# young-how/DQN-based-UAV-3D_path_planer

Measured on AMD Instinct MI355X. Metric: env-steps/sec + learner updates/sec, PathPlan_City DQN, higher is better.
Workload: dtype f64

## Files before the change

dqn_based_uav_3d_path_planer_amd/csrc/learner.hip:

```cpp
#include <hip/hip_runtime.h>
#include <hip/hip_fp16.h>
#include <stdint.h>
#include <stdlib.h>

#include "../../include/uavenv.h"
#include "uavenv_device.hpp"
#include "qnet_device.hpp"
#include "dqn_internal.hpp"
#include "dqn_slots_internal.hpp"

using namespace uav;
using namespace uavq;

namespace {

struct GradArgs {
    UavReplayRing ring;
    int head, filled, batch;
    uint64_t seed, counter;
    ReplayPerm perm;
    const int32_t *explicit_idx;
    const float *local, *target;
    int n_actions, dueling, kind;
    float gamma;
// ... 685 lines not shown
            csc = mfma16(ones ? 1.0f : xs[q][i], dh[q][i], csc);
            cw2 = mfma16(hh[q][i], bo[q][i], cw2);
        }
#pragma unroll
    for (int k = 0; k < 4; ++k) { A.acc[0][k] += csc[k]; A.acc[1][k] += cw2[k]; }
}

template <bool FIRST, bool GLDS>
__device__ __forceinline__ void grad_tile_packed8(const GradArgs &g, const GradLdsP &L, float *qn_lds, int tile, bool more,
                                                  GradAcc8 &A)
{
    constexpr int NMAX = 4;
    const int tid = (int)threadIdx.x, lane = tid & 63, wv = __builtin_amdgcn_readfirstlane(tid >> 6), grp = wv >> 2, strip = wv & 3;
    const int r = lane & 15, gq = lane >> 4, t256 = tid & 255;
    const int n2 = g.n_actions + (g.dueling ? 1 : 0);
    const uint32_t *obs = reinterpret_cast<const uint32_t *>(g.ring.obs);
    const float *net = grp == 0 ? g.local : g.target;
    floatx4 vW[kStageIters];
    SplitScRegs vS;
    float pw[4] = {0, 0, 0, 0}, pb2 = 0.0f;
    if (FIRST) {
        if (GLDS) img_glds(grp == 0 ? L.W1l : L.W1t, g.img + (grp == 0 ? 0 : kSplitF), strip);
        else if (g.img) img_issue(vW, g.img + (grp == 0 ? 0 : kSplitF));
        else w_issue_half(vW, net, t256);
        const NetDev nv = net_view(net, n2);
        if (!GLDS && !g.img) w_issue_sc(vS, net, nv.b1);
#pragma unroll
        for (int k = 0; k < 4; ++k) pw[k] = nv.W2[t256 + 256 * k < n2 * kHid ? t256 + 256 * k : 0];
        pb2 = nv.b2[t256 < n2 ? t256 : 0];
    }
    L_STAMP2(0);
    const int smp = tile * kTile + strip * 16 + r;
    int f, agent;
    if (g.explicit_idx) {
        f = g.explicit_idx[2 * smp];
        agent = g.explicit_idx[2 * smp + 1];
    } else {
        replay_slot_to_frame(g.perm, replay_perm_apply(g.perm, (uint32_t)smp), g.head, g.ring.frames, f, agent);
    }
    int fn = f + 1;
    if (fn >= g.ring.frames) fn = 0;
    const uint32_t row_s = (uint32_t)f * (uint32_t)g.ring.n_agents + (uint32_t)agent;
    const uint32_t row_n = (uint32_t)fn * (uint32_t)g.ring.n_agents + (uint32_t)agent;
    L_STAMP2(1);
    PRow R;
    prow_load(R, obs + (size_t)(grp == 0 ? row_s : row_n) * kPackedDwords);
    int p_act = 0;
    float p_rew = 0.0f, p_w = 1.0f;
    uint32_t raw_done = 0u, raw_valid = 1u;
    if (grp == 0) {
        load_transition(g.ring, row_s, p_act, p_rew, raw_done, raw_valid);
        p_w = g.is_w ? g.is_w[smp] : 1.0f;
    }
    L_STAMP(6);
    if (FIRST) {
        if (!GLDS) {
            if (g.img) img_commit(grp == 0 ? L.W1l : L.W1t, vW); else w_commit_split(w1split_at(grp == 0 ? L.W1l : L.W1t), vW, vS);
        }
        L_STAMP(7);
        float *W2 = grp == 0 ? L.W2l : L.W2t, *b2 = grp == 0 ? L.b2l : L.b2t;
#pragma unroll
        for (int k = 0; k < 4; ++k)
            if (t256 + 256 * k < n2 * kHid) W2[t256 + 256 * k] = pw[k];
        if (t256 < n2) b2[t256] = pb2;
        __syncthreads();
    }
    L_STAMP(1);
    floatx4 hl[4];
    W2Frag<NMAX> Fl;
    float ql[NMAX];
    if (grp == 0) {
        fwd_strip_split<false>(w1split_at(L.W1l), R, hl);
        w2_load<NMAX>(Fl, L.W2l, L.b2l, n2);
        q_strip<NMAX>(hl, Fl, n2, g.n_actions, g.dueling, ql);
        if (gq == 0) prow_store_lds(L.Ps + (strip * 16 + r) * kPackedDwords, R);
    } else {
        int best = 0;
        floatx4 ht[4];
        if (g.kind == 1) {
            fwd_strip_split<false>(w1split_at(L.W1l), R, ht);
            W2Frag<NMAX> F;
            w2_load<NMAX>(F, L.W2l, L.b2l, n2);
            float qn_l[NMAX];
            q_strip<NMAX>(ht, F, n2, g.n_actions, g.dueling, qn_l);
            float bq = qn_l[0];
#pragma unroll
            for (int a = 1; a < NMAX; ++a)
                if (a < g.n_actions && qn_l[a] > bq) { bq = qn_l[a]; best = a; }
        }
        fwd_strip_split<false>(w1split_at(L.W1t), R, ht);
        W2Frag<NMAX> Ft;
        w2_load<NMAX>(Ft, L.W2t, L.b2t, n2);
        float qt[NMAX];
        q_strip<NMAX>(ht, Ft, n2, g.n_actions, g.dueling, qt);
        if (gq == 0) qn_lds[strip * 16 + r] = pick_qn<NMAX>(g, qt, best);
    }
    L_STAMP(2);
    __syncthreads();
    L_STAMP(3);
    FlagOps FO;
    if (grp == 1) flag_ops_build(L, r, gq, FO);
    if (grp == 0) {
        GradAcc<NMAX> T;
#pragma unroll
        for (int a = 0; a < NMAX + 2; ++a) T.csum[a] = A.csum[a];
        float amax = 0.0f;
// ... 510 lines not shown
                if (grp == 0) A.acc[3] = mfma16h(*reinterpret_cast<const half8 *>(xa + 16 * 6 * kLdT + 32 * kk), bdh, A.acc[3]);
                else A.acc[3] = mfma16h(*reinterpret_cast<const half8 *>(ha + 32 * kk), *reinterpret_cast<const half8 *>(ob + 32 * kk), A.acc[3]);
            }
        }
        if (i + 1 < n_my) __syncthreads();
    }
    L_STAMP(5);
    grad_write_partials8(g, ga.stride, red, A);
}

constexpr size_t kGradH8Lds = (size_t)(4 * kTile * kLdH + 2 * kTile * kLdT + 2 * 112 * kLdT + 16 * kLdT) * 2 +
                              (size_t)(2 * kMaxOut * kHid + 2 * kMaxOut + 4 * (kMaxOut + 2) + 2 * kTile + 8 * kStageW) * 4;

template <typename ObsT, int NMAX>
__global__ void __launch_bounds__(256) k_dqn_grad(Grad2Args ga)
{
    const GradArgs &g = ga.g;
    extern __shared__ __align__(16) float lds[];
    GradLds L;
    L.W1l = lds;
    L.W1t = L.W1l + kTileF;
    L.Xs = L.W1t + kTileF;
    L.Xn = L.Xs + kTileF;
    L.dHs = L.Xn + kTileF;
    L.douts = L.dHs + kTile * kLh;
    L.W2l = L.douts + kTile * kMaxOut;
    L.W2t = L.W2l + kMaxOut * kHid;
    L.b2l = L.W2t + kMaxOut * kHid;
    L.b2t = L.b2l + kMaxOut;
    L.red = L.b2t + kMaxOut;
    const int tid = (int)threadIdx.x, lane = tid & 63, wv = tid >> 6, r = lane & 15, gq = lane >> 4;
    const int n2 = g.n_actions + (g.dueling ? 1 : 0);
    GradAcc<NMAX> A;
    A.acc2 = floatx4{0.0f, 0.0f, 0.0f, 0.0f};
#pragma unroll
    for (int u = 0; u < 7; ++u) A.acc1[u] = floatx4{0.0f, 0.0f, 0.0f, 0.0f};
#pragma unroll
    for (int a = 0; a < NMAX + 2; ++a) A.csum[a] = 0.0f;

    L_STAMP(0);
    const int step = (int)gridDim.x;
    int tile = (int)blockIdx.x;
    grad_tile<ObsT, NMAX, true>(g, L, tile, tile + step < ga.n_tiles, A);
    for (tile += step; tile < ga.n_tiles; tile += step)
        grad_tile<ObsT, NMAX, false>(g, L, tile, tile + step < ga.n_tiles, A);
    L_STAMP(5);
    grad_write_partials<NMAX>(g, ga.stride, L.red, A);
}

constexpr int kMaxGradGrid = 256;
constexpr size_t kGrad2Lds = (size_t)(4 * kTileF + kTile * kLh + kTile * kMaxOut + 2 * kMaxOut * kHid + 2 * kMaxOut +
                                      4 * (kMaxOut + 2)) * 4;

__device__ __forceinline__ float reduce_columns(const float *__restrict__ partials, int nblk, int P, int stride, float &c_out)
{
    __shared__ float red[32][33];
    __shared__ float red2[8][33];
    const int tid = (int)threadIdx.x;
    const int cg = tid & 7, rg = tid >> 3;
    const int p4 = (int)blockIdx.x * 32 + cg * 4;
    const bool col_ok = p4 < stride;
    floatx4 acc = floatx4{0.0f, 0.0f, 0.0f, 0.0f};
    float c = 0.0f;
    for (int b0 = 0; b0 < nblk; b0 += 256) {
        floatx4 t[8];
#pragma unroll
        for (int k = 0; k < 8; ++k) {
            const int b = b0 + rg + 32 * k;
            const int bb = b < nblk ? b : nblk - 1;
            t[k] = *reinterpret_cast<const floatx4 *>(partials + (size_t)bb * stride + (col_ok ? p4 : 0));
        }
        const int bc = b0 + tid;
        const float cv = partials[(size_t)(bc < nblk ? bc : nblk - 1) * stride + P + 1];
        c += bc < nblk ? cv : 0.0f;
#pragma unroll
        for (int k = 0; k < 8; ++k) {
            const bool ok = b0 + rg + 32 * k < nblk;
#pragma unroll
            for (int e = 0; e < 4; ++e) acc[e] += ok ? t[k][e] : 0.0f;
        }
    }
    c_out = c;
#pragma unroll
    for (int e = 0; e < 4; ++e) red[rg][cg * 4 + e] = acc[e];
    __syncthreads();
    {
        const int px = tid & 31, part = tid >> 5;
        red2[part][px] = (red[4 * part][px] + red[4 * part + 1][px]) + (red[4 * part + 2][px] + red[4 * part + 3][px]);
    }
    __syncthreads();
    float t = 0.0f;
    if (tid < 32) {
#pragma unroll
        for (int k = 0; k < 8; ++k) t += red2[k][tid];
    }
    return t;
}

__global__ void __launch_bounds__(256) k_dqn_reduce(const float *__restrict__ partials, int nblk, int P, int stride,
                                                    float *__restrict__ raw)
{
    float c;
    const float t = reduce_columns(partials, nblk, P, stride, c);
    const int p = (int)blockIdx.x * 32 + (int)threadIdx.x;
    if (threadIdx.x < 32 && p < P + 2) raw[p] = t;
}

__global__ void k_dqn_adam(float *__restrict__ local, float *__restrict__ target, float *__restrict__ m,
                           float *__restrict__ v, const float *__restrict__ raw, int P, float lr, float beta1,
                           float beta2, float eps, float bc1, float bc2_sqrt, int hard_update, float *__restrict__ loss,
                           float *__restrict__ img)
{
    const int p = (int)(blockIdx.x * blockDim.x + threadIdx.x);
    const float cnt = raw[P + 1];
    const float inv = 1.0f / (cnt > 1.0f ? cnt : 1.0f);
    if (p == 0 && loss) *loss = raw[P] * inv;
    if (p >= P) return;
    const float gp = raw[p] * inv;
    const float mp = m[p] + (gp - m[p]) * (1.0f - beta1);
    const float vp = v[p] * beta2 + (1.0f - beta2) * gp * gp;
    m[p] = mp;
    v[p] = vp;
    const float denom = sqrtf(vp) / bc2_sqrt + eps;
    const float np = local[p] - (lr / bc1) * (mp / denom);
    local[p] = np;
    if (hard_update) target[p] = np;
    if (img) {
        img_store_param(img, p, np);
        if (hard_update) img_store_param(img + kSplitF, p, np);
    }
}

__global__ void __launch_bounds__(256) k_dqn_reduce_adam(const float *__restrict__ partials, int nblk, int P, int stride,
                                                         float *__restrict__ local, float *__restrict__ target,
                                                         float *__restrict__ m, float *__restrict__ v, float lr,
                                                         float beta1, float beta2, float eps, float bc1, float bc2_sqrt,
                                                         int hard_update, float *__restrict__ loss, float *__restrict__ raw,
                                                         const uint32_t *__restrict__ go_word, uint32_t go_value, float *__restrict__ img)
{
    UAV_HOT_PRIO();
    if (go_word && __hip_atomic_load(go_word, __ATOMIC_RELAXED, __HIP_MEMORY_SCOPE_AGENT) != go_value) return;
    __shared__ float cnt_part[4];
    const int tid = (int)threadIdx.x;
    const int p = (int)blockIdx.x * 32 + tid;
    float m0 = 0.0f, v0 = 0.0f, w0 = 0.0f;
    if (tid < 32 && p < P) { m0 = m[p]; v0 = v[p]; w0 = local[p]; }
    float c;
    const float t = reduce_columns(partials, nblk, P, stride, c);
    for (int off = 32; off > 0; off >>= 1) c += __shfl_down(c, off, 64);
    if ((tid & 63) == 0) cnt_part[tid >> 6] = c;
    __syncthreads();
    const float cnt = (cnt_part[0] + cnt_part[1]) + (cnt_part[2] + cnt_part[3]);
    const float inv = 1.0f / (cnt > 1.0f ? cnt : 1.0f);
    if (tid < 32 && p < P + 2) {
        if (raw) raw[p] = t;
        if (p < P) {
            const float gp = t * inv;
            const float mp = m0 + (gp - m0) * (1.0f - beta1);
            const float vp = v0 * beta2 + (1.0f - beta2) * gp * gp;
            m[p] = mp;
            v[p] = vp;
            const float np = w0 - (lr / bc1) * (mp / (sqrtf(vp) / bc2_sqrt + eps));
            local[p] = np;
            if (hard_update) target[p] = np;
            if (img) {
                img_store_param(img, p, np);
                if (hard_update) img_store_param(img + kSplitF, p, np);
            }
        } else if (p == P && loss) {
            *loss = t * inv;
        }
    }
}

struct AdamSlotsArgs {
    int nblk, P, stride;
    float lr, beta1, beta2, eps;
    const uint32_t *go_word;
    uint32_t go_value;
    struct {
        const float *partials;
        float *local, *target, *m, *v, *loss, *raw, *img;
        float bc1, bc2_sqrt;
        int hard_update;
    } slot[kActMaxSlots];
};

__global__ void __launch_bounds__(256) k_dqn_reduce_adam_slots(AdamSlotsArgs a)
{
    const auto &sl = a.slot[blockIdx.y];
    const float *__restrict__ partials = sl.partials;
    float *__restrict__ local = sl.local, *__restrict__ target = sl.target, *__restrict__ m = sl.m, *__restrict__ v = sl.v;
    float *__restrict__ loss = sl.loss, *__restrict__ raw = sl.raw, *__restrict__ img = sl.img;
    const uint32_t *__restrict__ go_word = a.go_word;
    const uint32_t go_value = a.go_value;
    const int nblk = a.nblk, P = a.P, stride = a.stride, hard_update = sl.hard_update;
    const float lr = a.lr, beta1 = a.beta1, beta2 = a.beta2, eps = a.eps, bc1 = sl.bc1, bc2_sqrt = sl.bc2_sqrt;
    UAV_HOT_PRIO();
    if (go_word && __hip_atomic_load(go_word, __ATOMIC_RELAXED, __HIP_MEMORY_SCOPE_AGENT) != go_value) return;
    __shared__ float cnt_part[4];
    const int tid = (int)threadIdx.x;
    const int p = (int)blockIdx.x * 32 + tid;
    float m0 = 0.0f, v0 = 0.0f, w0 = 0.0f;
    if (tid < 32 && p < P) { m0 = m[p]; v0 = v[p]; w0 = local[p]; }
    float c;
    const float t = reduce_columns(partials, nblk, P, stride, c);
    for (int off = 32; off > 0; off >>= 1) c += __shfl_down(c, off, 64);
    if ((tid & 63) == 0) cnt_part[tid >> 6] = c;
    __syncthreads();
    const float cnt = (cnt_part[0] + cnt_part[1]) + (cnt_part[2] + cnt_part[3]);
    const float inv = 1.0f / (cnt > 1.0f ? cnt : 1.0f);
    if (tid < 32 && p < P + 2) {
        if (raw) raw[p] = t;
        if (p < P) {
            const float gp = t * inv;
            const float mp = m0 + (gp - m0) * (1.0f - beta1);
            const float vp = v0 * beta2 + (1.0f - beta2) * gp * gp;
            m[p] = mp;
            v[p] = vp;
            const float np = w0 - (lr / bc1) * (mp / (sqrtf(vp) / bc2_sqrt + eps));
            local[p] = np;
            if (hard_update) target[p] = np;
            if (img) {
                img_store_param(img, p, np);
                if (hard_update) img_store_param(img + kSplitF, p, np);
            }
        } else if (p == P && loss) {
            *loss = t * inv;
        }
    }
}

struct ActArgs {
    const void *obs;
    int n, n_actions, dueling;
    const float *local;
    float eps;
    uint64_t seed, counter;
    int32_t *index_out;
    float *steer_out;
    float *q_out;
    const float *img;
};

template <typename ObsT, int NMAX>
__global__ void __launch_bounds__(256) k_dqn_act(ActArgs g)
{
    extern __shared__ __align__(16) float lds[];
    float *W1 = lds;
    float *Xs = W1 + kTileF;
    float *W2 = Xs + kTileF;
    float *b2 = W2 + kMaxOut * kHid;
    const int tid = (int)threadIdx.x, lane = tid & 63, wv = tid >> 6, r = lane & 15;
    const int n2 = g.n_actions + (g.dueling ? 1 : 0);
    const NetDev nl = net_view(g.local, n2);
    const int first = (int)blockIdx.x * kTile + wv * 16;
    float *strip = Xs + wv * kStripF;
    floatx4 vX[kXIters], vW[kStageIters];
    {
// ... 736 lines not shown
```

dqn_based_uav_3d_path_planer_amd/csrc/qnet_device.hpp:

```cpp
#pragma once
#include <hip/hip_runtime.h>
#include <stdint.h>

#include "uavenv_device.hpp"

namespace uavq {

using namespace uav;

constexpr int kW = 100;
constexpr int kHid = 64;
constexpr int kTile = 64;
constexpr int kMaxOut = 16;

struct NetDev {
    const float *W1, *b1, *W2, *b2;
};

__device__ __forceinline__ NetDev net_view(const float *flat, int n2)
{
    NetDev n;
    n.W1 = flat;
    n.b1 = flat + kHid * kW;
    n.W2 = n.b1 + kHid;
// ... 288 lines not shown
#pragma unroll
    for (int it = 0; it < kStageIters; ++it)
#pragma unroll
        for (int e = 0; e < 4; ++e) {
            h[it][e] = (_Float16)v[it][e];
            m[it][e] = (_Float16)((v[it][e] - (float)h[it][e]) * 2048.0f);
        }
#pragma unroll
    for (int it = 0; it < kStageIters; ++it) {
        const int c = it * 256 + tid;
        const int row = c / 25, q = c - row * 25;
        if (c < kStageChunks && q >= 2 && q < 24) {
            *reinterpret_cast<half4 *>(S.hi + row * kLdHs + 4 * q - kFlagC0) = h[it];
            *reinterpret_cast<half4 *>(S.mid + row * kLdHs + 4 * q - kFlagC0) = m[it];
        }
    }
    float *d = S.sc + (tid >> 2) * kScK + 5 * (tid & 3);
#pragma unroll
    for (int i = 0; i < 5; ++i) d[i] = R.v[i];
}
__device__ __forceinline__ void stage_actor_split(const W1Split &S, const float *flat)
{
    floatx4 v[kStageIters];
    SplitScRegs sc;
    w_issue(v, flat);
    w_issue_sc(sc, flat, flat + kHid * kW);
    w_commit_split(S, v, sc);
}
constexpr int kImgPieces = kSplitBytes / 16;
static_assert((kImgPieces + 255) / 256 == kStageIters, "the image is staged through the registers of w_issue");
__device__ __forceinline__ void img_issue(floatx4 (&v)[kStageIters], const float *img)
{
    const int tid = (int)threadIdx.x & 255;
#pragma unroll
    for (int it = 0; it < kStageIters; ++it) {
        int c = it * 256 + tid;
        c = c < kImgPieces ? c : kImgPieces - 1;
        v[it] = *reinterpret_cast<const floatx4 *>(img + 4 * c);
    }
}
__device__ __forceinline__ void img_commit(float *lds_image, const floatx4 (&v)[kStageIters])
{
    const int tid = (int)threadIdx.x & 255;
#pragma unroll
    for (int it = 0; it < kStageIters; ++it) {
        const int c = it * 256 + tid;
        if (c < kImgPieces) *reinterpret_cast<floatx4 *>(lds_image + 4 * c) = v[it];
    }
}
__device__ __forceinline__ void glds16(const void *src, void *lds_base)
{
    __builtin_amdgcn_global_load_lds((__attribute__((address_space(1))) void *)src,
                                     (__attribute__((address_space(3))) void *)lds_base, 16, 0, 0);
}
constexpr int kImgDma = kImgPieces / 64;
static_assert(kImgPieces % 64 == 0 && (kImgDma + 3) / 4 == 7 && kImgDma > 4 * 6, "the image is 27 whole wavefront-instructions");
__device__ __forceinline__ void img_glds(float *lds_image, const float *img, int w)
{
    const int lane = (int)threadIdx.x & 63;
#pragma unroll
    for (int it = 0; it < 6; ++it) {
        const int c = (4 * it + w) * 64;
        glds16(img + 4 * (c + lane), lds_image + 4 * c);
    }
    const int c = (24 + w) * 64;
    if (c < kImgPieces) glds16(img + 4 * (c + lane), lds_image + 4 * c);
}
__device__ __forceinline__ void img_store_param(float *img, int p, float w)
{
    const W1Split S = w1split_at(img);
    if (p < kHid * kW) {
        const int row = p / kW;
        split_store(S, row, p - row * kW, w);
    } else if (p < kHid * kW + kHid) {
        S.sc[(p - kHid * kW) * kScK + 15] = w;
    }
}

__device__ __forceinline__ half8 bits_to_half8(uint32_t byte)
{
    uintx4 d;
#pragma unroll
    for (int k = 0; k < 4; ++k)
        d[k] = ((byte >> (2 * k)) & 1u ? 0x3c00u : 0u) | ((byte >> (2 * k + 1)) & 1u ? 0x3c000000u : 0u);
    return *reinterpret_cast<const half8 *>(&d);
}
__device__ __forceinline__ uint32_t flag_byte(const PRow &R, int kk, int g)
{
    const uint32_t lo = kk == 0 ? R.m0 : (kk == 1 ? R.m1 : R.m2), hi = kk == 0 ? R.m1 : (kk == 1 ? R.m2 : 0u);
    return g == 3 ? (hi & 0xffu) : ((lo >> (8 * (g + 1))) & 0xffu);
}
__device__ __forceinline__ int flag_aoff(int kk, int g)
{
    return (kk == 2 && g == 3) ? 0 : 32 * kk + 8 * g;
}
__device__ __forceinline__ float sel4(float a0, float a1, float a2, float a3, uint32_t m1, uint32_t m2)
{
    const uint32_t lo = (__float_as_uint(a1) & m1) | (__float_as_uint(a0) & ~m1);
    const uint32_t hi = (__float_as_uint(a3) & m1) | (__float_as_uint(a2) & ~m1);
    return __uint_as_float((hi & m2) | (lo & ~m2));
}

template <bool EXT>
__device__ __forceinline__ void fwd_strip_split_ahead(const W1Split &S, const PRow &R, floatx4 (&acc)[4], float e0 = 0.0f, float e1 = 0.0f)
{
    const int lane = (int)threadIdx.x & 63, r = lane & 15, g = lane >> 4;
// ... 265 lines not shown
```

dqn_based_uav_3d_path_planer_amd/csrc/uavenv.hip:

```cpp
#include <hip/hip_runtime.h>

#include <algorithm>
#include <cmath>
#include <cstdarg>
#include <cstdio>
#include <cstdlib>
#include <cstring>
#include <map>
#include <mutex>
#include <new>
#include <utility>
#include <vector>

#include "../../include/uavenv.h"
#include "uavenv_device.hpp"
#include "qnet_device.hpp"
#include "dqn_internal.hpp"

using namespace uav;

extern "C" int uavenv_rrt_plan_at(UavEnv *env, int32_t first, int32_t m, const double *start_goal_dev, const double *uniforms_dev,
                                  int32_t stream_len, uint64_t seed, int32_t max_iter, double step_size, double obstacle_step,
                                  double *out_start_goal_dev, double *out_sub_dev, int32_t *out_nsub_dev,
                                  int32_t *out_iters_dev, void *node_scratch, int32_t scratch_wgs, void *stream);
// ... 979 lines not shown
    const DevState &S = a.st;
    const int N = a.N;
    const int lane = (int)threadIdx.x & 63, wv = __builtin_amdgcn_readfirstlane((int)threadIdx.x >> 6);
    const int first = (int)blockIdx.x * 64;
    const int i = first + lane;
    const bool active = i < N;
    const int ii = active ? i : N - 1;
    CoopLds *C = reinterpret_cast<CoopLds *>(smem + a.obsq_off);
    const bool want_obs = a.obs && !(a.flags & UAVENV_STEP_NO_OBS);
    const bool auto_reset = (a.flags & UAVENV_STEP_AUTO_RESET) != 0;
    UAV_CSTAMP(0);

    const uavq::W1Split pW1 = uavq::w1split_at(reinterpret_cast<float *>(smem + a.pol_off));
    float *pW2 = reinterpret_cast<float *>(smem + a.pol_off) + uavq::kSplitF;
    float *pb2 = pW2 + uavq::kMaxOut * uavq::kHid;
    int32_t *pact = reinterpret_cast<int32_t *>(pb2 + uavq::kMaxOut);
    uavq::floatx4 vW[uavq::kStageIters];
    uavq::PRow prow;
    uavq::SplitScRegs pol_sc;
    float pol_w2[4] = {0, 0, 0, 0}, pol_b2v = 0.0f;
    uint4 pol_rn = make_uint4(0u, 0u, 0u, 0u);
    const int pol_i = first + wv * 16 + (lane & 15);
    const int pol_n2 = a.n_actions + (a.pol_dueling ? 1 : 0);
    if (POLICY) {
        const int tid = (int)threadIdx.x;
        const uavq::NetDev nl = uavq::net_view(a.pol_local, pol_n2);
        if (GLDS) {
            uavq::img_glds(reinterpret_cast<float *>(smem + a.pol_off), a.pol_img, wv);
            if (wv >= 2) stage_copy_glds(smem, a, wv - 2, 2);
        } else if (a.pol_img) uavq::img_issue(vW, a.pol_img);
        else { uavq::w_issue(vW, a.pol_local); uavq::w_issue_sc(pol_sc, a.pol_local, nl.b1); }
#pragma unroll
        for (int k = 0; k < 4; ++k) pol_w2[k] = nl.W2[tid + 256 * k < pol_n2 * uavq::kHid ? tid + 256 * k : pol_n2 * uavq::kHid - 1];
        pol_b2v = nl.b2[tid < pol_n2 ? tid : 0];
        uavq::prow_load(prow, a.pol_obs + (size_t)(pol_i < N ? pol_i : N - 1) * kPackedDwords);
        pol_rn = philox4x32_10(make_uint4((uint32_t)pol_i, (uint32_t)a.pol_counter, (uint32_t)(a.pol_counter >> 32), 0xac7u),
                               make_uint2((uint32_t)a.pol_seed, (uint32_t)(a.pol_seed >> 32)));
    }
    Agent g;
    RawAction ra = {0u, 0u};
    double head_old = 0.0;
    uint32_t meta_a1 = 0u;
    if (wv == 0) {
        load_agent(S, ii, g);
        if (!POLICY) ra = load_action_raw(a.actions, a.action_kind, ii);
        if (a.meta_a1) meta_a1 = __float_as_uint(a.meta_a1[ii]);
    } else if (wv == 2) {
        head_old = S.F(F_HEAD)[ii];
        if (!POLICY) ra = load_action_raw(a.actions, a.action_kind, ii);
    }
    ResetCand cand;
    double cand_heading = 0.0;
    bool cand_want = false;
    if (wv == 1 && auto_reset) {
        const int c_flags = S.I(I_FLAGS)[ii], c_sub = S.I(I_SUBIDX)[ii], c_n = S.I(I_NTOTAL)[ii], c_step = S.I(I_STEP)[ii];
        const double dx = S.F(F_GX)[ii] - S.F(F_PX)[ii], dy = S.F(F_GY)[ii] - S.F(F_PY)[ii],
                     dz = S.F(F_GZ)[ii] - S.F(F_PZ)[ii];
        cand_heading = reset_candidate_draw(a, ii, cand);
        const double reach = 7.0 + a.max_v + 1.0;
        cand_want = (c_flags & kFlagDone) || c_sub >= c_n - 1 || c_step + 1 >= a.max_step ||
                    dx * dx + dy * dy + dz * dz < reach * reach;
        if (cand_want) reset_candidate_fetch(a, cand);
    }
    uint2 lut[7];
    {
        const int lo = wv == 0 ? 0 : 7 + (wv - 1) * 6;
#pragma unroll
        for (int j = 0; j < 6; ++j) lut[j] = a.emit_lut[(lo + j) * 64 + lane];
        lut[6] = a.emit_lut[6 * 64 + lane];
    }
    uint32_t *trow = C->tile + lane * kCTileLd;
    if (wv == 3) { trow[0] = 0u; trow[1] = 0u; trow[2] = 0u; }
    double r = 0.0, a0 = 0.0;
    int ret_done = 0, info = UAVENV_INFO_NORMAL, valid = 1, agent_done = 0;
    double energy = 0.0;
    bool did_reset = false, skip = false, head_set = false;
    PreStep pre;
    pre.moved = false;
    if (POLICY) {
        const int tid = (int)threadIdx.x;
        if (!GLDS) {
            if (a.pol_img) uavq::img_commit(reinterpret_cast<float *>(smem + a.pol_off), vW); else uavq::w_commit_split(pW1, vW, pol_sc);
        }
#pragma unroll
        for (int k = 0; k < 4; ++k) {
            const int at = tid + 256 * k < pol_n2 * uavq::kHid ? tid + 256 * k : pol_n2 * uavq::kHid - 1;
            pW2[at] = pol_w2[k];
        }
        if (tid < pol_n2) pb2[tid] = pol_b2v;
    }
    if (wv >= 2) {
        if (!(POLICY && GLDS)) stage_copy(smem, a, (int)threadIdx.x - 128, 128);
    } else if (wv == 0) {
        unpack_flags(g);
        const bool masked = a.active && a.active[ii] == 0;
        skip = masked || ((a.flags & UAVENV_STEP_SKIP_DONE) && g.done);
        if (!POLICY) {
            a0 = decode_action(ra, a.action_kind, a.n_actions);
            if (!skip) step_pre(a, a0, g, pre);
        }
        else if (!skip) {
            step_pre_dists(g, pre);
        }
    }
    __syncthreads();
    UAV_PSTAMP(1);
    const WorldLds<MaskT> w = world_view<MaskT>(smem, a);
    if (POLICY) {
        uavq::floatx4 h[4];
        uavq::W2Frag<4> F;
        if (PAHEAD) uavq::fwd_strip_split_ahead<false>(pW1, prow, h);
        else uavq::fwd_strip_split<false>(pW1, prow, h);
        UAV_PSTAMP(2);
        float q[4];
        uavq::w2_load<4>(F, pW2, pb2, pol_n2);
        uavq::q_strip<4>(h, F, pol_n2, a.n_actions, a.pol_dueling, q);
        if (lane < 16) {
            const float sample = (float)(pol_rn.x >> 8) * (1.0f / 16777216.0f);
            int act;
            if (sample > a.pol_eps) {
                act = 0;
                float bq = q[0];
#pragma unroll
                for (int k = 1; k < 4; ++k)
                    if (k < a.n_actions && q[k] > bq) { bq = q[k]; act = k; }
            } else {
                act = (int)(((uint64_t)pol_rn.y * (uint64_t)a.n_actions) >> 32);
            }
            pact[wv * 16 + lane] = act;
            if (pol_i < N) a.pol_act[pol_i] = act;
        }
        UAV_PSTAMP(3);
        __syncthreads();
        UAV_PSTAMP(4);
        if (wv == 0 || wv == 2) ra.lo = (uint32_t)pact[lane];
        if (wv == 0) {
            a0 = decode_action(ra, UAVENV_ACT_INDEX_I32, a.n_actions);
            if (!skip && pre.moved) {
                double sn, cs;
                sincos(g.head + a0 * a.steer, &sn, &cs);
                step_pre_move(a, g, pre, sn, cs);
            }
        }
// ... 300 lines not shown
    c.scn = row;
    reset_candidate_fetch(a, c);
    double vx, vy;
    if (v.v0) {
        vx = v.v0[(size_t)L.e * 2];
        vy = v.v0[(size_t)L.e * 2 + 1];
    } else {
        const uint4 r = philox4x32_10(make_uint4((uint32_t)L.e, 0u, 0u, 0xe7a1u), make_uint2((uint32_t)v.seed, (uint32_t)(v.seed >> 32)));
        double sn, cs;
        sincos(kTwoPi * u53(r.x, r.y), &sn, &cs);
        vx = a.max_v * cs;
        vy = a.max_v * sn;
    }
    L.v0x = vx;
    L.v0y = vy;
    c.f[14] = calc_v(vx, vy, a.max_v);
    c.f[12] = vx;
    c.f[13] = vy;
    c.f[15] = angle_of<true>(vx, vy);
    apply_reset<APF>(a, APF ? li : L.e, g, c);
    L.steps = 0;
    L.collisions = 0;
    L.cap = c.n_total * a.max_step + 1;
    L.ret = 0.0;
    L.energy = 0.0;
    if (v.traj_steps > 0) {
        double *p = v.traj_pos + (size_t)L.e * (v.traj_steps + 1) * 3;
        p[0] = g.o.px; p[1] = g.o.py; p[2] = g.o.pz;
    }
}

template <typename MaskT>
__global__ void __launch_bounds__(256, 1) k_eval_episodes(StepArgs a, EvalArgs v)
{
    extern __shared__ __align__(16) unsigned char smem[];
    const int lane = (int)threadIdx.x & 63, wv = __builtin_amdgcn_readfirstlane((int)threadIdx.x >> 6);
    const int tid = (int)threadIdx.x;
    float *img = reinterpret_cast<float *>(smem + v.img_off);
    float *W2 = reinterpret_cast<float *>(smem + v.w2_off);
    float *b2 = W2 + uavq::kMaxOut * uavq::kHid;
    uavq::img_glds(img, v.img, wv);
    if (wv >= 2) stage_copy_glds(smem, a, wv - 2, 2);
    {
        const uavq::NetDev nl = uavq::net_view(v.local, v.n2);
#pragma unroll
        for (int k = 0; k < 4; ++k)
            if (tid + 256 * k < v.n2 * uavq::kHid) W2[tid + 256 * k] = nl.W2[tid + 256 * k];
        if (tid < v.n2) b2[tid] = nl.b2[tid];
    }
    Agent g = {};
    EvalLane L = {};
    L.e = (int)blockIdx.x * 256 + tid;
    bool install = true;
    __syncthreads();
    const WorldLds<MaskT> w = world_view<MaskT>(smem, a);
    const uavq::W1Split W1 = uavq::w1split_at(img);
    unsigned char *slot = smem + v.slot_off + wv * v.slot_bytes;
    ObsWaveLds *Q = reinterpret_cast<ObsWaveLds *>(slot);
    uint32_t *rows = reinterpret_cast<uint32_t *>(slot);
    const int r16 = lane & 15, grp = lane >> 4;
    const int A = a.n_actions;
    for (;;) {
        if (install) eval_install(a, v, g, L);
        install = false;
        if (__ballot(L.e < v.n) == 0ull) break;
        const bool have = L.e < v.n;
        const ObsBits bits = obs_bits_queued(w, Q, g.o.px, g.o.py, g.o.pz, have);
        const ObsScalars sc = obs_scalars(g.o, g.head);
        uavq::PRow R;
        ctile_mask_words(bits, R.m0, R.m1, R.m2);
#pragma unroll
        for (int k = 0; k < 11; ++k) R.sc[k] = sc.f[k];
#pragma unroll
        for (int k = 0; k < 4; ++k) R.sg[k] = sc.f[11 + k];
        if (!have) {
            R.m0 = R.m1 = R.m2 = 0u;
#pragma unroll
            for (int k = 0; k < 11; ++k) R.sc[k] = 0.0f;
#pragma unroll
            for (int k = 0; k < 4; ++k) R.sg[k] = 0.0f;
        }
        wave_lds_sync();
        uavq::prow_store_lds(rows + lane * kPackedDwords, R);
        wave_lds_sync();
        float q[4] = {0.0f, 0.0f, 0.0f, 0.0f};
#pragma unroll 1
        for (int st = 0; st < 4; ++st) {
            uavq::PRow Rs;
            uavq::prow_load(Rs, rows + (16 * st + r16) * kPackedDwords);
            uavq::floatx4 h[4];
            uavq::fwd_strip_split<false>(W1, Rs, h);
            uavq::W2Frag<4> F;
            uavq::w2_load<4>(F, W2, b2, v.n2);
            float qs[4];
            uavq::q_strip<4>(h, F, v.n2, A, v.dueling, qs);
#pragma unroll
            for (int k = 0; k < 4; ++k) q[k] = grp == st ? qs[k] : q[k];
        }
        wave_lds_sync();
        if (have) {
            int act = 0;
            float bq = q[0];
#pragma unroll
            for (int k = 1; k < 4; ++k)
                if (k < A && q[k] > bq) { bq = q[k]; act = k; }
            if (v.eps > 0.0f) {
// ... 43 lines not shown
    float bound;
    int32_t mode, n_actors;
    int32_t n, first, max_steps, traj_steps, lanes;
    int32_t img_off, w2_off, slot_off, slot_bytes;
};

__device__ __forceinline__ float2 eval_sac_noise(uint64_t seed, int e, int step)
{
    const uint4 r = philox4x32_10(make_uint4((uint32_t)e, (uint32_t)step, 0u, 0x5ac0u), make_uint2((uint32_t)seed, (uint32_t)(seed >> 32)));
    const float u1 = ((float)(r.x >> 8) + 1.0f) * (1.0f / 16777216.0f);
    const float u2 = (float)(r.y >> 8) * (1.0f / 16777216.0f);
    const float rad = sqrtf(-2.0f * logf(u1));
    float sn, cs;
    sincosf(6.283185307179586f * u2, &sn, &cs);
    return make_float2(rad * cs, rad * sn);
}

__global__ void __launch_bounds__(256) k_eval_noise_fill(uint64_t seed, int n, int steps, float *__restrict__ out)
{
    const int64_t total = (int64_t)n * steps;
    for (int64_t i = (int64_t)blockIdx.x * 256 + threadIdx.x; i < total; i += (int64_t)gridDim.x * 256) {
        const int e = (int)(i / steps);
        const float2 z = eval_sac_noise(seed, e, (int)(i - (int64_t)e * steps));
        out[2 * i] = z.x;
        out[2 * i + 1] = z.y;
    }
}

template <typename MaskT, bool APF>
__global__ void __launch_bounds__(256, 1) k_eval_episodes_sac(StepArgs a, SacEvalArgs v)
{
    extern __shared__ __align__(16) unsigned char smem[];
    const int lane = (int)threadIdx.x & 63, wv = __builtin_amdgcn_readfirstlane((int)threadIdx.x >> 6);
    const int tid = (int)threadIdx.x;
    const int y = (int)blockIdx.y;
    const float *actor = v.actor[y];
    float *W2 = reinterpret_cast<float *>(smem + v.w2_off);
    float *b2 = W2 + 4 * uavq::kHid;
    const uavq::W1Split W1 = uavq::w1split_at(reinterpret_cast<float *>(smem + v.img_off));
    if (wv >= 2) stage_copy_glds(smem, a, wv - 2, 2);
    {
        const uavq::NetDev nl = uavq::net_view(actor, 4);
        const float w2v = nl.W2[tid];
        const float b2v = nl.b2[tid & 3];
        uavq::stage_actor_split(W1, actor);
        W2[tid] = w2v;
        if (tid < 4) b2[tid] = b2v;
    }
    Agent g = {};
    EvalLane L = {};
    const int li = ((int)blockIdx.y * (int)gridDim.x + (int)blockIdx.x) * 256 + tid;
    L.e = y + v.n_actors * ((int)blockIdx.x * 256 + tid);
    bool install = true;
    __syncthreads();
    const WorldLds<MaskT> w = world_view<MaskT>(smem, a);
    unsigned char *slot = smem + v.slot_off + wv * v.slot_bytes;
    ObsWaveLds *Q = reinterpret_cast<ObsWaveLds *>(slot);
    uint32_t *rows = reinterpret_cast<uint32_t *>(slot);
    const int r16 = lane & 15, grp = lane >> 4;
    for (;;) {
        if (install) eval_install<APF>(a, v, g, L, li);
        install = false;
        if (__ballot(L.e < v.n) == 0ull) break;
        const bool have = L.e < v.n;
        const ObsBits bits = obs_bits_queued(w, Q, g.o.px, g.o.py, g.o.pz, have);
        const ObsScalars sc = obs_scalars(g.o, g.head);
        uavq::PRow R;
        ctile_mask_words(bits, R.m0, R.m1, R.m2);
#pragma unroll
        for (int k = 0; k < 11; ++k) R.sc[k] = sc.f[k];
#pragma unroll
        for (int k = 0; k < 4; ++k) R.sg[k] = sc.f[11 + k];
        if (!have) {
            R.m0 = R.m1 = R.m2 = 0u;
#pragma unroll
            for (int k = 0; k < 11; ++k) R.sc[k] = 0.0f;
#pragma unroll
            for (int k = 0; k < 4; ++k) R.sg[k] = 0.0f;
        }
        wave_lds_sync();
        uavq::prow_store_lds(rows + lane * kPackedDwords, R);
        wave_lds_sync();
        float o[4] = {0.0f, 0.0f, 0.0f, 0.0f};
#pragma unroll 1
        for (int st = 0; st < 4; ++st) {
            uavq::PRow Rs;
            uavq::prow_load(Rs, rows + (16 * st + r16) * kPackedDwords);
            uavq::floatx4 h[4];
            uavq::fwd_strip_split<false>(W1, Rs, h);
            uavq::W2Frag<4> F;
            uavq::w2_load<4>(F, W2, b2, 4);
            float os[4];
            uavq::q_strip<4>(h, F, 4, 4, 0, os);
#pragma unroll
            for (int k = 0; k < 4; ++k) o[k] = grp == st ? os[k] : o[k];
        }
        wave_lds_sync();
        if (have) {
            float2 z = make_float2(0.0f, 0.0f);
            if (v.mode == UAVENV_EVAL_SAC_SAMPLE) z = eval_sac_noise(v.seed, L.e, L.steps);
            const float act0 = uavq::actor_head_one(o[0], o[2], z.x).act * v.bound;
            const int j = L.e % a.U;
            const double a0 = decode_action(RawAction{__float_as_uint(act0), 0u}, UAVENV_ACT_STEER_F32, a.n_actions);
            PreStep P;
            step_pre(a, a0, g, P);
            if (P.moved) g.head = angle_of<true>(g.o.vx, g.o.vy);
// ... 12 lines not shown
                const float act1 = uavq::actor_head_one(o[1], o[3], z.y).act * v.bound;
                reinterpret_cast<float2 *>(v.traj_act)[(size_t)L.e * v.traj_steps + L.steps - 1] = make_float2(act0, act1);
            }
            const bool trunc = (v.max_steps > 0 && L.steps >= v.max_steps) || L.steps >= L.cap;
            if (g.done || trunc) {
                const int outcome = g.done ? (info == UAVENV_INFO_LOSE ? UAVENV_EVAL_LOSE : UAVENV_EVAL_SUCCESS) : UAVENV_EVAL_TRUNCATED;
                eval_store_record(v, L.e, g, L, outcome, j);
                L.e += v.lanes;
                install = true;
            }
        }
    }
}

struct SlotsEvalArgs {
    const float *local[UAVENV_SAC_LOOP_MAX_SLOTS];
    const float *img;
    const double *v0;
    uint4 *rec;
    double *traj_pos;
    int8_t *traj_act;
    uint64_t seed;
    float eps;
    int32_t n_nets;
    int32_t n, first, max_steps, traj_steps, lanes;
    int32_t n2, dueling;
    int32_t img_off, w2_off, slot_off, slot_bytes;
};

template <typename MaskT, bool APF>
__global__ void __launch_bounds__(256, 1) k_eval_episodes_slots(StepArgs a, SlotsEvalArgs v)
{
    extern __shared__ __align__(16) unsigned char smem[];
    const int lane = (int)threadIdx.x & 63, wv = __builtin_amdgcn_readfirstlane((int)threadIdx.x >> 6);
    const int tid = (int)threadIdx.x;
    const int y = (int)blockIdx.y;
    float *img = reinterpret_cast<float *>(smem + v.img_off);
    float *W2 = reinterpret_cast<float *>(smem + v.w2_off);
    float *b2 = W2 + uavq::kMaxOut * uavq::kHid;
    uavq::img_glds(img, v.img + (size_t)y * uavq::kSplitF, wv);
    if (wv >= 2) stage_copy_glds(smem, a, wv - 2, 2);
    {
        const uavq::NetDev nl = uavq::net_view(v.local[y], v.n2);
#pragma unroll
        for (int k = 0; k < 4; ++k)
            if (tid + 256 * k < v.n2 * uavq::kHid) W2[tid + 256 * k] = nl.W2[tid + 256 * k];
        if (tid < v.n2) b2[tid] = nl.b2[tid];
    }
    Agent g = {};
    EvalLane L = {};
    const int li = ((int)blockIdx.y * (int)gridDim.x + (int)blockIdx.x) * 256 + tid;
    L.e = y + v.n_nets * ((int)blockIdx.x * 256 + tid);
    bool install = true;
    __syncthreads();
    const WorldLds<MaskT> w = world_view<MaskT>(smem, a);
    const uavq::W1Split W1 = uavq::w1split_at(img);
    unsigned char *slot = smem + v.slot_off + wv * v.slot_bytes;
    ObsWaveLds *Q = reinterpret_cast<ObsWaveLds *>(slot);
    uint32_t *rows = reinterpret_cast<uint32_t *>(slot);
    const int r16 = lane & 15, grp = lane >> 4;
    const int A = a.n_actions;
    for (;;) {
        if (install) eval_install<APF>(a, v, g, L, li);
        install = false;
        if (__ballot(L.e < v.n) == 0ull) break;
        const bool have = L.e < v.n;
        const ObsBits bits = obs_bits_queued(w, Q, g.o.px, g.o.py, g.o.pz, have);
        const ObsScalars sc = obs_scalars(g.o, g.head);
        uavq::PRow R;
        ctile_mask_words(bits, R.m0, R.m1, R.m2);
#pragma unroll
        for (int k = 0; k < 11; ++k) R.sc[k] = sc.f[k];
#pragma unroll
        for (int k = 0; k < 4; ++k) R.sg[k] = sc.f[11 + k];
        if (!have) {
            R.m0 = R.m1 = R.m2 = 0u;
#pragma unroll
            for (int k = 0; k < 11; ++k) R.sc[k] = 0.0f;
#pragma unroll
            for (int k = 0; k < 4; ++k) R.sg[k] = 0.0f;
        }
        wave_lds_sync();
        uavq::prow_store_lds(rows + lane * kPackedDwords, R);
        wave_lds_sync();
        float q[4] = {0.0f, 0.0f, 0.0f, 0.0f};
#pragma unroll 1
        for (int st = 0; st < 4; ++st) {
            uavq::PRow Rs;
            uavq::prow_load(Rs, rows + (16 * st + r16) * kPackedDwords);
            uavq::floatx4 h[4];
            uavq::fwd_strip_split<false>(W1, Rs, h);
            uavq::W2Frag<4> F;
            uavq::w2_load<4>(F, W2, b2, v.n2);
            float qs[4];
            uavq::q_strip<4>(h, F, v.n2, A, v.dueling, qs);
#pragma unroll
            for (int k = 0; k < 4; ++k) q[k] = grp == st ? qs[k] : q[k];
        }
        wave_lds_sync();
        if (have) {
            int act = 0;
            float bq = q[0];
#pragma unroll
            for (int k = 1; k < 4; ++k)
                if (k < A && q[k] > bq) { bq = q[k]; act = k; }
            if (v.eps > 0.0f) {
// ... 1245 lines not shown
```

Before: 626.1 million.

## Add explicit global-to-LDS waits, defer go-flag check, reorder reset candidate loads

Adds an explicit vmcnt wait after global_load_lds DMA before the barrier in several kernels, so the LDS data is complete when read rather than relying on implicit ordering. The go-word check in the reduce+Adam kernels moves to after the first partial loads have been issued, so the early-exit test overlaps with memory latency instead of gating it. The environment step kernel splits the reset-candidate logic: state loads are issued early, the random draw and predicate are computed after the LUT loads, and the candidate fetch happens after the policy weight staging. This aims to hide load latency, but the added waits could serialize and the later early exit wastes some loads.

```diff
diff --git a/dqn_based_uav_3d_path_planer_amd/csrc/learner.hip b/dqn_based_uav_3d_path_planer_amd/csrc/learner.hip
--- a/dqn_based_uav_3d_path_planer_amd/csrc/learner.hip
+++ b/dqn_based_uav_3d_path_planer_amd/csrc/learner.hip
@@ -761,6 +761,7 @@
         load_transition(g.ring, row_s, p_act, p_rew, raw_done, raw_valid);
         p_w = g.is_w ? g.is_w[smp] : 1.0f;
     }
+    if (FIRST && GLDS) glds_wait();
     L_STAMP(6);
     if (FIRST) {
         if (!GLDS) {
@@ -1377,7 +1378,9 @@
 constexpr size_t kGrad2Lds = (size_t)(4 * kTileF + kTile * kLh + kTile * kMaxOut + 2 * kMaxOut * kHid + 2 * kMaxOut +
                                       4 * (kMaxOut + 2)) * 4;
 
-__device__ __forceinline__ float reduce_columns(const float *__restrict__ partials, int nblk, int P, int stride, float &c_out)
+template <bool GATED>
+__device__ __forceinline__ float reduce_columns_gated(const float *__restrict__ partials, int nblk, int P, int stride, float &c_out,
+                                                      const uint32_t *go_word, uint32_t go_value, bool &go)
 {
     __shared__ float red[32][33];
     __shared__ float red2[8][33];
@@ -1398,6 +1401,13 @@
         const int bc = b0 + tid;
         const float cv = partials[(size_t)(bc < nblk ? bc : nblk - 1) * stride + P + 1];
         c += bc < nblk ? cv : 0.0f;
+        if (GATED && b0 == 0 && go_word) {
+            asm volatile("" ::: "memory");
+            if (__hip_atomic_load(go_word, __ATOMIC_RELAXED, __HIP_MEMORY_SCOPE_AGENT) != go_value) {
+                go = false;
+                return 0.0f;
+            }
+        }
 #pragma unroll
         for (int k = 0; k < 8; ++k) {
             const bool ok = b0 + rg + 32 * k < nblk;
@@ -1420,6 +1430,11 @@
         for (int k = 0; k < 8; ++k) t += red2[k][tid];
     }
     return t;
+}
+__device__ __forceinline__ float reduce_columns(const float *__restrict__ partials, int nblk, int P, int stride, float &c_out)
+{
+    bool go = true;
+    return reduce_columns_gated<false>(partials, nblk, P, stride, c_out, nullptr, 0u, go);
 }
 
 __global__ void __launch_bounds__(256) k_dqn_reduce(const float *__restrict__ partials, int nblk, int P, int stride,
@@ -1464,14 +1479,15 @@
                                                          const uint32_t *__restrict__ go_word, uint32_t go_value, float *__restrict__ img)
 {
     UAV_HOT_PRIO();
-    if (go_word && __hip_atomic_load(go_word, __ATOMIC_RELAXED, __HIP_MEMORY_SCOPE_AGENT) != go_value) return;
     __shared__ float cnt_part[4];
     const int tid = (int)threadIdx.x;
     const int p = (int)blockIdx.x * 32 + tid;
     float m0 = 0.0f, v0 = 0.0f, w0 = 0.0f;
     if (tid < 32 && p < P) { m0 = m[p]; v0 = v[p]; w0 = local[p]; }
     float c;
-    const float t = reduce_columns(partials, nblk, P, stride, c);
+    bool go = true;
+    const float t = reduce_columns_gated<true>(partials, nblk, P, stride, c, go_word, go_value, go);
+    if (!go) return;
     for (int off = 32; off > 0; off >>= 1) c += __shfl_down(c, off, 64);
     if ((tid & 63) == 0) cnt_part[tid >> 6] = c;
     __syncthreads();
@@ -1522,14 +1538,15 @@
     const int nblk = a.nblk, P = a.P, stride = a.stride, hard_update = sl.hard_update;
     const float lr = a.lr, beta1 = a.beta1, beta2 = a.beta2, eps = a.eps, bc1 = sl.bc1, bc2_sqrt = sl.bc2_sqrt;
     UAV_HOT_PRIO();
-    if (go_word && __hip_atomic_load(go_word, __ATOMIC_RELAXED, __HIP_MEMORY_SCOPE_AGENT) != go_value) return;
     __shared__ float cnt_part[4];
     const int tid = (int)threadIdx.x;
     const int p = (int)blockIdx.x * 32 + tid;
     float m0 = 0.0f, v0 = 0.0f, w0 = 0.0f;
     if (tid < 32 && p < P) { m0 = m[p]; v0 = v[p]; w0 = local[p]; }
     float c;
-    const float t = reduce_columns(partials, nblk, P, stride, c);
+    bool go = true;
+    const float t = reduce_columns_gated<true>(partials, nblk, P, stride, c, go_word, go_value, go);
+    if (!go) return;
     for (int off = 32; off > 0; off >>= 1) c += __shfl_down(c, off, 64);
     if ((tid & 63) == 0) cnt_part[tid >> 6] = c;
     __syncthreads();
diff --git a/dqn_based_uav_3d_path_planer_amd/csrc/qnet_device.hpp b/dqn_based_uav_3d_path_planer_amd/csrc/qnet_device.hpp
--- a/dqn_based_uav_3d_path_planer_amd/csrc/qnet_device.hpp
+++ b/dqn_based_uav_3d_path_planer_amd/csrc/qnet_device.hpp
@@ -364,6 +364,10 @@
 {
     __builtin_amdgcn_global_load_lds((__attribute__((address_space(1))) void *)src,
                                      (__attribute__((address_space(3))) void *)lds_base, 16, 0, 0);
+}
+__device__ __forceinline__ void glds_wait()
+{
+    __builtin_amdgcn_s_waitcnt(0x0f70);
 }
 constexpr int kImgDma = kImgPieces / 64;
 static_assert(kImgPieces % 64 == 0 && (kImgDma + 3) / 4 == 7 && kImgDma > 4 * 6, "the image is 27 whole wavefront-instructions");
diff --git a/dqn_based_uav_3d_path_planer_amd/csrc/uavenv.hip b/dqn_based_uav_3d_path_planer_amd/csrc/uavenv.hip
--- a/dqn_based_uav_3d_path_planer_amd/csrc/uavenv.hip
+++ b/dqn_based_uav_3d_path_planer_amd/csrc/uavenv.hip
@@ -1055,15 +1055,13 @@
     ResetCand cand;
     double cand_heading = 0.0;
     bool cand_want = false;
-    if (wv == 1 && auto_reset) {
-        const int c_flags = S.I(I_FLAGS)[ii], c_sub = S.I(I_SUBIDX)[ii], c_n = S.I(I_NTOTAL)[ii], c_step = S.I(I_STEP)[ii];
-        const double dx = S.F(F_GX)[ii] - S.F(F_PX)[ii], dy = S.F(F_GY)[ii] - S.F(F_PY)[ii],
-                     dz = S.F(F_GZ)[ii] - S.F(F_PZ)[ii];
-        cand_heading = reset_candidate_draw(a, ii, cand);
-        const double reach = 7.0 + a.max_v + 1.0;
-        cand_want = (c_flags & kFlagDone) || c_sub >= c_n - 1 || c_step + 1 >= a.max_step ||
-                    dx * dx + dy * dy + dz * dz < reach * reach;
-        if (cand_want) reset_candidate_fetch(a, cand);
+    const bool cand_wave = wv == 1 && auto_reset;
+    int c_flags = 0, c_sub = 0, c_n = 0, c_step = 0;
+    double c_gx = 0.0, c_gy = 0.0, c_gz = 0.0, c_px = 0.0, c_py = 0.0, c_pz = 0.0;
+    if (cand_wave) {
+        c_flags = S.I(I_FLAGS)[ii]; c_sub = S.I(I_SUBIDX)[ii]; c_n = S.I(I_NTOTAL)[ii]; c_step = S.I(I_STEP)[ii];
+        c_gx = S.F(F_GX)[ii]; c_gy = S.F(F_GY)[ii]; c_gz = S.F(F_GZ)[ii];
+        c_px = S.F(F_PX)[ii]; c_py = S.F(F_PY)[ii]; c_pz = S.F(F_PZ)[ii];
     }
     uint2 lut[7];
     {
@@ -1071,6 +1069,15 @@
 #pragma unroll
         for (int j = 0; j < 6; ++j) lut[j] = a.emit_lut[(lo + j) * 64 + lane];
         lut[6] = a.emit_lut[6 * 64 + lane];
+    }
+    if (cand_wave) {
+        cand_heading = reset_candidate_draw(a, ii, cand);
+        asm volatile("" : "+v"(c_flags), "+v"(c_sub), "+v"(c_n), "+v"(c_step));
+        asm volatile("" : "+v"(c_gx), "+v"(c_gy), "+v"(c_gz), "+v"(c_px), "+v"(c_py), "+v"(c_pz));
+        const double dx = c_gx - c_px, dy = c_gy - c_py, dz = c_gz - c_pz;
+        const double reach = 7.0 + a.max_v + 1.0;
+        cand_want = ((c_flags & kFlagDone) != 0) | (c_sub >= c_n - 1) | (c_step + 1 >= a.max_step) |
+                    (dx * dx + dy * dy + dz * dz < reach * reach);
     }
     uint32_t *trow = C->tile + lane * kCTileLd;
     if (wv == 3) { trow[0] = 0u; trow[1] = 0u; trow[2] = 0u; }
@@ -1085,6 +1092,7 @@
         if (!GLDS) {
             if (a.pol_img) uavq::img_commit(reinterpret_cast<float *>(smem + a.pol_off), vW); else uavq::w_commit_split(pW1, vW, pol_sc);
         }
+        if (GLDS) uavq::glds_wait();
 #pragma unroll
         for (int k = 0; k < 4; ++k) {
             const int at = tid + 256 * k < pol_n2 * uavq::kHid ? tid + 256 * k : pol_n2 * uavq::kHid - 1;
@@ -1092,6 +1100,7 @@
         }
         if (tid < pol_n2) pb2[tid] = pol_b2v;
     }
+    if (cand_wave && cand_want) reset_candidate_fetch(a, cand);
     if (wv >= 2) {
         if (!(POLICY && GLDS)) stage_copy(smem, a, (int)threadIdx.x - 128, 128);
     } else if (wv == 0) {
@@ -1498,6 +1507,7 @@
     EvalLane L = {};
     L.e = (int)blockIdx.x * 256 + tid;
     bool install = true;
+    uavq::glds_wait();
     __syncthreads();
     const WorldLds<MaskT> w = world_view<MaskT>(smem, a);
     const uavq::W1Split W1 = uavq::w1split_at(img);
@@ -1647,6 +1657,7 @@
     const int li = ((int)blockIdx.y * (int)gridDim.x + (int)blockIdx.x) * 256 + tid;
     L.e = y + v.n_actors * ((int)blockIdx.x * 256 + tid);
     bool install = true;
+    uavq::glds_wait();
     __syncthreads();
     const WorldLds<MaskT> w = world_view<MaskT>(smem, a);
     unsigned char *slot = smem + v.slot_off + wv * v.slot_bytes;
@@ -1765,6 +1776,7 @@
     const int li = ((int)blockIdx.y * (int)gridDim.x + (int)blockIdx.x) * 256 + tid;
     L.e = y + v.n_nets * ((int)blockIdx.x * 256 + tid);
     bool install = true;
+    uavq::glds_wait();
     __syncthreads();
     const WorldLds<MaskT> w = world_view<MaskT>(smem, a);
     const uavq::W1Split W1 = uavq::w1split_at(img);
```

Measured after the change: 626.1 million (median of 2 runs). About the same (-0.0%).
